# jianzhnie/ScaleRL

Measured on NVIDIA H100. Metric: learner_frames_per_sec, higher is better.
Workload: dtype bf16

## Files before the change

scalerl_b200/csrc/common.cuh:

```cuda
#pragma once
#include <cuda_runtime.h>
#include <cuda_bf16.h>
#include <stdint.h>
#include "wgmma.cuh"

#define SRL_DEVINL __device__ __forceinline__

#ifndef SRL_SPIN_LIMIT
#define SRL_SPIN_LIMIT (1u << 24)
#endif

namespace srl {

SRL_DEVINL uint32_t smem_u32(const void* p) { return static_cast<uint32_t>(__cvta_generic_to_shared(p)); }

SRL_DEVINL void mbar_init(uint64_t* bar, uint32_t count) {
  asm volatile("mbarrier.init.shared::cta.b64 [%0], %1;" ::"r"(smem_u32(bar)), "r"(count) : "memory");
}
SRL_DEVINL void mbar_fence_init() { asm volatile("fence.mbarrier_init.release.cluster;" ::: "memory"); }
SRL_DEVINL void mbar_arrive(uint64_t* bar) {
  asm volatile("{\n\t.reg .b64 st;\n\tmbarrier.arrive.shared::cta.b64 st, [%0];\n\t}" ::"r"(smem_u32(bar)) : "memory");
}
SRL_DEVINL void mbar_arrive_expect_tx(uint64_t* bar, uint32_t bytes) {
  asm volatile("{\n\t.reg .b64 st;\n\tmbarrier.arrive.expect_tx.shared::cta.b64 st, [%0], %1;\n\t}" ::"r"(smem_u32(bar)), "r"(bytes)
               : "memory");
}
SRL_DEVINL bool mbar_try_wait(uint64_t* bar, uint32_t parity) {
  uint32_t ok;
  asm volatile(
      "{\n\t.reg .pred p;\n\t"
      "mbarrier.try_wait.parity.shared::cta.b64 p, [%1], %2;\n\t"
      "selp.u32 %0, 1, 0, p;\n\t}"
      : "=r"(ok)
      : "r"(smem_u32(bar)), "r"(parity)
      : "memory");
  return ok != 0;
}
SRL_DEVINL void mbar_wait(uint64_t* bar, uint32_t parity) {
  uint32_t spins = 0;
  while (!mbar_try_wait(bar, parity)) {
    if (++spins > SRL_SPIN_LIMIT) { __trap(); }
  }
}

#ifdef SRL_KSTAMP
static __device__ unsigned long long* g_kstamp = nullptr;
SRL_DEVINL unsigned long long kstamp_now() { unsigned long long t; asm volatile("mov.u64 %0, %%globaltimer;" : "=l"(t)); return t; }
SRL_DEVINL void kstamp_put(int kid, unsigned long long t0) {
  if (g_kstamp && blockIdx.x == 0 && blockIdx.y == 0 && threadIdx.x == 0) {
    const unsigned long long t1 = kstamp_now(), i = atomicAdd(g_kstamp, 1ull);
    if (i < 2000) { g_kstamp[1 + 3 * i] = (unsigned long long)kid; g_kstamp[2 + 3 * i] = t0; g_kstamp[3 + 3 * i] = t1; }
  }
}
#define SRL_KSTAMP_SETTER(fn) void fn(unsigned long long* q) { cudaMemcpyToSymbol(g_kstamp, &q, sizeof q); }
#else
#define SRL_KSTAMP_SETTER(fn) void fn(unsigned long long*) {}
#endif
SRL_DEVINL void pdl_wait(int kid = 0) {
#ifdef SRL_KSTAMP
  const unsigned long long t0 = kstamp_now();
#endif
  asm volatile("griddepcontrol.wait;" ::: "memory");
#ifdef SRL_KSTAMP
  if (kid) kstamp_put(kid, t0);
#else
  (void)kid;
#endif
}
SRL_DEVINL void pdl_launch() { asm volatile("griddepcontrol.launch_dependents;" ::: "memory"); }

SRL_DEVINL uint4 lds128(uint32_t saddr) {
  uint4 v;
  asm volatile("ld.shared.v4.b32 {%0, %1, %2, %3}, [%4];" : "=r"(v.x), "=r"(v.y), "=r"(v.z), "=r"(v.w) : "r"(saddr) : "memory");
  return v;
}
SRL_DEVINL void sts_volatile_f32(uint32_t saddr, float v) { asm volatile("st.volatile.shared.f32 [%0], %1;" ::"r"(saddr), "f"(v) : "memory"); }

SRL_DEVINL void fence_proxy_async_smem() { asm volatile("fence.proxy.async.shared::cta;" ::: "memory"); }

SRL_DEVINL uint32_t elect_one_sync() {
  uint32_t pred;
  __syncwarp();
  asm volatile("{\n\t.reg .pred P;\n\telect.sync _|P, 0xffffffff;\n\tselp.u32 %0, 1, 0, P;\n\t}" : "=r"(pred));
  return pred;
}
SRL_DEVINL void wg_fence() { asm volatile("wgmma.fence.sync.aligned;" ::: "memory"); }
SRL_DEVINL void wg_commit() { asm volatile("wgmma.commit_group.sync.aligned;" ::: "memory"); }
SRL_DEVINL void wg_wait_all() { asm volatile("wgmma.wait_group.sync.aligned 0;" ::: "memory"); }
SRL_DEVINL void wg_wait_prev() { asm volatile("wgmma.wait_group.sync.aligned 1;" ::: "memory"); }
template <int N> SRL_DEVINL void reg_release() { asm volatile("setmaxnreg.dec.sync.aligned.u32 %0;" ::"n"(N)); }
template <int N> SRL_DEVINL void reg_claim() { asm volatile("setmaxnreg.inc.sync.aligned.u32 %0;" ::"n"(N)); }
template <int N>
SRL_DEVINL void wg_fence_regs(float (&d)[N]) {
#pragma unroll
  for (int i = 0; i < N; ++i) asm volatile("" : "+f"(d[i])::"memory");
}
SRL_DEVINL void named_bar(int id, int threads) { asm volatile("bar.sync %0, %1;" ::"r"(id), "r"(threads) : "memory"); }

template <int N, int TA, int TB>
SRL_DEVINL void wg_mma128(float (&d)[2][N / 2], uint64_t ad, uint32_t a_hi, uint64_t bd, uint32_t accumulate) {
  Wgmma<N, TA, TB>::mma(d[0], ad, bd, accumulate);
  Wgmma<N, TA, TB>::mma(d[1], ad + a_hi, bd, accumulate);
}

constexpr int fit_stages(int want, int fixed, int per) {
  int s = want;
  while (s > 1 && fixed + s * per > 232448) --s;
  return s;
}
constexpr int WG_IMG_STRIDE = 20;
constexpr int WG_IMG_BYTES = 2 * 128 * WG_IMG_STRIDE * 4;
template <int N, bool ONE_BUF = false>
SRL_DEVINL void wg_acc_rows16(const float (&d0)[N / 2], const float (&d1)[N / 2], int c, float* img, int wt, int bar, float (&v)[16]) {
  float* buf = ONE_BUF ? img : img + (c & 1) * 128 * WG_IMG_STRIDE;
  if (ONE_BUF) named_bar(bar, 128);
  const int w = wt >> 5, l = wt & 31;
#pragma unroll
  for (int h = 0; h < 2; ++h)
#pragma unroll
    for (int jj = 0; jj < 2; ++jj)
#pragma unroll
      for (int rr = 0; rr < 2; ++rr) {
        const int row = 64 * h + 16 * w + (l >> 2) + 8 * rr, i = 4 * (2 * c + jj) + 2 * rr;
        const float (&d)[N / 2] = h ? d1 : d0;
        *reinterpret_cast<float2*>(buf + row * WG_IMG_STRIDE + 8 * jj + 2 * (l & 3)) = make_float2(d[i], d[i + 1]);
      }
  named_bar(bar, 128);
  const float4* q = reinterpret_cast<const float4*>(buf + wt * WG_IMG_STRIDE);
#pragma unroll
  for (int j = 0; j < 4; ++j) { const float4 x = q[j]; v[4 * j] = x.x; v[4 * j + 1] = x.y; v[4 * j + 2] = x.z; v[4 * j + 3] = x.w; }
}
template <int N, bool ONE_BUF = false>
SRL_DEVINL void wg_acc_row16(const float (&d)[2][N / 2], int c, float* img, int wt, int bar, float (&v)[16]) {
  wg_acc_rows16<N, ONE_BUF>(d[0], d[1], c, img, wt, bar, v);
}

SRL_DEVINL uint64_t make_smem_desc(uint32_t saddr, uint32_t lbo_bytes, uint32_t sbo_bytes) {
  uint64_t d = 0;
  d |= (uint64_t)((saddr & 0x3FFFF) >> 4);
  d |= (uint64_t)((lbo_bytes >> 4) & 0x3FFF) << 16;
  d |= (uint64_t)((sbo_bytes >> 4) & 0x3FFF) << 32;
  d |= (uint64_t)1 << 62;
  return d;
}
SRL_DEVINL uint64_t make_smem_desc_sw64(uint32_t saddr, uint32_t lbo_bytes, uint32_t sbo_bytes) {
  return (make_smem_desc(saddr, lbo_bytes, sbo_bytes) & ~((uint64_t)3 << 62)) | ((uint64_t)2 << 62);
}

SRL_DEVINL uint32_t swz128(uint32_t row, uint32_t chunk) { return row * 128u + ((chunk ^ (row & 7u)) << 4); }
SRL_DEVINL uint32_t swz64(uint32_t row, uint32_t chunk) { return row * 64u + ((chunk ^ ((row >> 1) & 3u)) << 4); }

SRL_DEVINL uint32_t pack_bf16x2(float lo, float hi) {
  __nv_bfloat162 v = __floats2bfloat162_rn(lo, hi);
  return *reinterpret_cast<uint32_t*>(&v);
}
SRL_DEVINL float bf16_lo(uint32_t v) { return __uint_as_float(v << 16); }
SRL_DEVINL float bf16_hi(uint32_t v) { return __uint_as_float(v & 0xFFFF0000u); }

SRL_DEVINL void red_add_v4(float* addr, float a, float b, float c, float d) {
  asm volatile("red.global.add.v4.f32 [%0], {%1, %2, %3, %4};" ::"l"(addr), "f"(a), "f"(b), "f"(c), "f"(d) : "memory");
}
SRL_DEVINL void red_add_16(float* dst, const float (&v)[16], float scale = 1.0f) {
#pragma unroll
  for (int j = 0; j < 16; j += 4) red_add_v4(dst + j, v[j] * scale, v[j + 1] * scale, v[j + 2] * scale, v[j + 3] * scale);
}

SRL_DEVINL int ld_action(const int64_t* p, int A) {
  const long long a = __ldg(reinterpret_cast<const long long*>(p));
  return a < 0 ? 0 : (a >= A ? A - 1 : (int)a);
}

SRL_DEVINL float warp_sum(float v) {
#pragma unroll
  for (int o = 16; o > 0; o >>= 1) v += __shfl_xor_sync(0xffffffffu, v, o);
  return v;
}

SRL_DEVINL bool take_ticket(float* scratch) {
  __threadfence();
  return atomicAdd(reinterpret_cast<unsigned*>(scratch), 1u) == gridDim.x - 1;
}

}
```

scalerl_b200/csrc/encoder.cu:

```cuda
#include "encoder_problems.cuh"
#include "tma_problems.cuh"
#include "res_problems.cuh"
#include "enc_fused.cuh"
#include "kernels.h"
#include <stdio.h>
#include <stdlib.h>

namespace srl {

constexpr int PACK_BLOCKS_FK = 256, PACK_BLOCKS_FD = 256, PACK_BLOCKS_CONV = 288;
SRL_DEVINL void pack_store(bf16* __restrict__ out, bf16* __restrict__ out_lo, int64_t i, float v) {
  const bf16 hi = __float2bfloat16_rn(v);
  out[i] = hi;
  if (out_lo) out_lo[i] = __float2bfloat16_rn(v - __bfloat162float(hi));
}
SRL_DEVINL void pack_store2(bf16* __restrict__ out, bf16* __restrict__ out_lo, int64_t i, float v0, float v1) {
  const bf16 h0 = __float2bfloat16_rn(v0), h1 = __float2bfloat16_rn(v1);
  *reinterpret_cast<uint32_t*>(out + i) = pack_bf16x2(v0, v1);
  if (out_lo) *reinterpret_cast<uint32_t*>(out_lo + i) = pack_bf16x2(v0 - __bfloat162float(h0), v1 - __bfloat162float(h1));
}
__global__ void __launch_bounds__(256) pack_weights_kernel(ParamPtrs p, bf16* __restrict__ out, bf16* __restrict__ out_lo, int skip_w1k) {
  pdl_wait(2);
  __shared__ __align__(16) float tile[64 * 99];
  const int t = threadIdx.x, b = blockIdx.x;
// ... 44 lines not shown
      } else if (i < WPack::W3K) {
        const int e = (int)(i - WPack::W2K), co = e >> 9, k = e & 511, tap = k >> 5, c = k & 31;
        v = p.w2[((co * 32 + c) << 4) + tap];
      } else if (i < WPack::WFK) {
        const int e = (int)(i - WPack::W3K), co = e / 576, k = e - co * 576, tap = k >> 6, c = k & 63;
        v = p.w3[(co * 64 + c) * 9 + tap];
      } else if (i < WPack::W2D) {
        const int e = (int)(i - WPack::W3D), c = e / 576, k = e - c * 576, tap = k >> 6, co = k & 63;
        v = p.w3[(co * 64 + c) * 9 + tap];
      } else {
        const int e = (int)(i - WPack::W2D), cls = e >> 13, r = e & 8191, c = r >> 8, k = r & 255, tt = k >> 6, co = k & 63;
        const int kh = (cls >> 1) + 2 * (tt >> 1), kw = (cls & 1) + 2 * (tt & 1);
        v = p.w2[((co * 32 + c) << 4) + kh * 4 + kw];
      }
      pack_store(out, out_lo, i, v);
    }
  }
}

__global__ void __launch_bounds__(352) obs_s2d_kernel(const uint8_t* __restrict__ obs, bf16* __restrict__ xs, int frame_blocks,
                                                      const float* __restrict__ w1, bf16* __restrict__ w1k, bf16* __restrict__ w1k_lo) {
  pdl_wait(1);
  pdl_launch();
  if ((int)blockIdx.x >= frame_blocks) {
    const int e = ((int)blockIdx.x - frame_blocks) * 352 + (int)threadIdx.x;
    if (e < 32 * 256 && w1k) {
      const int co = e >> 8, k = e & 255, tap = k >> 6, q = k & 63;
      const int c = q >> 4, dy = (q >> 2) & 3, dx = q & 3, kh = 4 * (tap >> 1) + dy, kw = 4 * (tap & 1) + dx;
      pack_store(w1k, w1k_lo, e, __ldg(w1 + co * 256 + c * 64 + kh * 8 + kw));
    }
    return;
  }
  __shared__ uint32_t tile[21][16][21];
  const int n = blockIdx.x;
  const int t = threadIdx.x;
  if (t < 336) {
    const int g = t / 21, X = t - g * 21;
    const uint8_t* src = obs + (size_t)n * 28224 + (g >> 2) * 7056 + (g & 3) * 84;
#pragma unroll
    for (int y = 0; y < 21; ++y) tile[y][g][X] = __ldg(reinterpret_cast<const uint32_t*>(src + y * 336) + X);
  }
  __syncthreads();
  if (t < 336) {
    const int X = t >> 4, g = t & 15;
#pragma unroll
    for (int y = 0; y < 21; ++y) {
      const uint32_t w = tile[y][g][X];
      const float f0 = __uint_as_float(__byte_perm(w, 0x4B000000u, 0x7540)) - 8388608.f;
      const float f1 = __uint_as_float(__byte_perm(w, 0x4B000000u, 0x7541)) - 8388608.f;
      const float f2 = __uint_as_float(__byte_perm(w, 0x4B000000u, 0x7542)) - 8388608.f;
      const float f3 = __uint_as_float(__byte_perm(w, 0x4B000000u, 0x7543)) - 8388608.f;
      *reinterpret_cast<uint2*>(xs + (((size_t)n * 21 + y) * 21 + X) * 64 + g * 4) = make_uint2(pack_bf16x2(f0, f1), pack_bf16x2(f2, f3));
    }
  }
}

__global__ void __launch_bounds__(256) a3_transpose_kernel(const bf16* __restrict__ a3, bf16* __restrict__ a3t) {
  pdl_wait(53);
  __shared__ __align__(16) uint16_t tile[49 * 66];
  const int n = blockIdx.x, t = threadIdx.x;
  const uint4* src = reinterpret_cast<const uint4*>(a3 + (size_t)n * 3136);
  for (int q = t; q < 392; q += 256) {
    const uint4 v = __ldg(src + q);
    uint32_t* d = reinterpret_cast<uint32_t*>(tile + (q >> 3) * 66 + (q & 7) * 8);
    d[0] = v.x; d[1] = v.y; d[2] = v.z; d[3] = v.w;
  }
  __syncthreads();
  uint32_t* dst = reinterpret_cast<uint32_t*>(a3t + (size_t)n * 3136);
  for (int pp = t; pp < 1568; pp += 256) {
    const int o = 2 * pp, c0 = o / 49, h0 = o - c0 * 49, o1 = o + 1, c1 = o1 / 49, h1 = o1 - c1 * 49;
    dst[pp] = (uint32_t)tile[h0 * 66 + c0] | ((uint32_t)tile[h1 * 66 + c1] << 16);
  }
}
SRL_KSTAMP_SETTER(kstamp_set_encoder)

cudaError_t launch_a3_transpose(const bf16* a3, bf16* a3t, int frames, cudaStream_t st) {
  if (frames <= 0) return cudaSuccess;
  a3_transpose_kernel<<<frames, 256, 0, st>>>(a3, a3t);
  return cudaGetLastError();
}

cudaError_t launch_pack_weights(const ParamPtrs& p, bf16* wpack, cudaStream_t st, bf16* wpack_lo, bool skip_w1k) {
  pack_weights_kernel<<<PACK_BLOCKS_FK + PACK_BLOCKS_FD + PACK_BLOCKS_CONV, 256, 0, st>>>(p, wpack, wpack_lo, skip_w1k ? 1 : 0);
  return cudaGetLastError();
}

#define SRL_TRY(x) do { cudaError_t e_ = (x); if (e_ != cudaSuccess) return e_; } while (0)

static inline int cdiv(int a, int b) { return (a + b - 1) / b; }

typedef CUresult (*EncodeTiledFn)(CUtensorMap*, CUtensorMapDataType, cuuint32_t, void*, const cuuint64_t*, const cuuint64_t*,
                                  const cuuint32_t*, const cuuint32_t*, CUtensorMapInterleave, CUtensorMapSwizzle,
                                  CUtensorMapL2promotion, CUtensorMapFloatOOBfill);

static EncodeTiledFn encode_fn() {
  static EncodeTiledFn fn = nullptr;
  if (!fn) {
    void* f = nullptr;
    cudaDriverEntryPointQueryResult q;
    if (cudaGetDriverEntryPoint("cuTensorMapEncodeTiled", &f, cudaEnableDefault, &q) == cudaSuccess && q == cudaDriverEntryPointSuccess)
      fn = reinterpret_cast<EncodeTiledFn>(f);
  }
  return fn;
}

bool make_map(CUtensorMap* m, const void* base, int rank, const uint64_t* dims, const uint64_t* strides_elems, const uint32_t* box,
              bool swizzle64) {
  EncodeTiledFn fn = encode_fn();
  if (!fn) return false;
  cuuint64_t gd[5], gs[4];
  cuuint32_t bx[5], es[5];
  for (int i = 0; i < rank; ++i) { gd[i] = dims[i]; bx[i] = box[i]; es[i] = 1; }
  for (int i = 0; i + 1 < rank; ++i) gs[i] = strides_elems[i] * 2;
  return fn(m, CU_TENSOR_MAP_DATA_TYPE_BFLOAT16, (cuuint32_t)rank, const_cast<void*>(base), gd, gs, bx, es, CU_TENSOR_MAP_INTERLEAVE_NONE,
            swizzle64 ? CU_TENSOR_MAP_SWIZZLE_64B : CU_TENSOR_MAP_SWIZZLE_128B, CU_TENSOR_MAP_L2_PROMOTION_L2_128B,
            CU_TENSOR_MAP_FLOAT_OOB_FILL_NONE) == CUDA_SUCCESS;
}

struct MapBuilder {
  const char* failed = nullptr;
  bool lo = false, failed_lo = false;
  void operator()(CUtensorMap* m, const void* base, uint64_t inner, uint64_t rows, uint32_t box_inner, uint32_t box_rows, const char* name,
                  bool swizzle64 = false) {
    const uint64_t d[2] = {inner, rows}, s[1] = {inner};
    const uint32_t bx[2] = {box_inner, box_rows};
    if (!failed && !make_map(m, base, 2, d, s, bx, swizzle64)) { failed = name; failed_lo = lo; }
  }
};

static void build_operand_maps(MapBuilder& mk, const OperandTensors& b, uint64_t nf, uint64_t nb, OperandMaps* M) {
  mk(&M->a1p0_w, b.a1, 64, nf * 100, 64, RConv2Fwd::WROWS, "a1p0_w");
  mk(&M->a1p1_w, b.a1 + (size_t)nf * 100 * 64, 64, nf * 100, 64, RConv2Fwd::WROWS, "a1p1_w");
  mk(&M->a2_w, b.a2, 64, nf * 81, 64, RConv3Fwd::WROWS, "a2_w");
  mk(&M->da3g_w, b.da3, 64, nb * 81, 64, RConv3Dgrad::WROWS, "da3g_w");
  mk(&M->da3g_b, b.da3, 64, nb * 81, 64, 128, "da3g_b");
  mk(&M->da2g_w, b.da2, 64, nb * 100, 64, RConv2Dgrad::WROWS, "da2g_w");
  mk(&M->da2g_b, b.da2, 64, nb * 100, 64, 128, "da2g_b");
  mk(&M->da1g_b, b.da1, 32, nb * 441, 32, 128, "da1g_b", true);
  mk(&M->a3m128, b.a3, 3136, nf, 64, 128, "a3m128");
  mk(&M->a3m64, b.a3, 3136, nf, 64, 64, "a3m64");
  mk(&M->dhm128, b.dh, 512, nb, 64, 128, "dhm128");
  mk(&M->dhm64, b.dh, 512, nb, 64, 64, "dhm64");
  const bf16* w = b.wpack;
  mk(&M->w1k, w + WPack::W1K, 256, 32, 64, 32, "w1k");
  mk(&M->w2k, w + WPack::W2K, 512, 64, 64, 64, "w2k");
  mk(&M->w3k, w + WPack::W3K, 576, 64, 64, 64, "w3k");
  mk(&M->wfk, w + WPack::WFK, 3136, 512, 64, 64, "wfk");
  mk(&M->wfd, w + WPack::WFD, 512, 3136, 64, 64, "wfd");
  mk(&M->w3d, w + WPack::W3D, 576, 64, 64, 64, "w3d");
  mk(&M->w2d, w + WPack::W2D, 256, 128, 64, 128, "w2d");
}

cudaError_t build_tma_maps(const EncoderBuffers& b, int NF, int NB, TmaMaps* M, const char** why) {
  static_assert(RConv1Wgrad::WROWS == RConv1Fwd::WROWS && RConv2Wgrad::WROWS == RConv2Fwd::WROWS && RConv3Wgrad::WROWS == RConv3Fwd::WROWS,
                "forward and wgrad share the window maps");
  const uint64_t nf = NF, nb = NB;
  MapBuilder mk;
  mk(&M->xs_w, b.xs, 64, nf * 441, 64, RConv1Fwd::WROWS, "xs_w");
  mk(&M->a3tm64, b.a3t, 3136, nf, 64, 64, "a3tm64");
  build_operand_maps(mk, b.hi, nf, nb, &M->hi);
  mk.lo = true;
  if (b.lo.wpack) build_operand_maps(mk, b.lo, nf, nb, &M->lo);
  M->valid = !mk.failed;
  if (mk.failed && why) {
    static thread_local char name[32];
    snprintf(name, sizeof(name), "%s%s", mk.failed, mk.failed_lo ? "_lo" : "");
    *why = name;
  }
  return mk.failed ? cudaErrorInvalidValue : cudaSuccess;
}

static cudaError_t launch_s2d(const uint8_t* obs, int frames, bf16* xs, cudaStream_t st, const float* w1, bf16* w1k, bf16* w1k_lo) {
  constexpr int WB = (32 * 256 + 351) / 352;
  SRL_TRY(launch_chain(obs_s2d_kernel, dim3(frames + WB), dim3(352), 0, st, obs, xs, frames, w1, w1k, w1k_lo));
  return cudaGetLastError();
}

static int sm_count() {
  static const int n = [] { int d = 0, v = 0; cudaGetDevice(&d); cudaDeviceGetAttribute(&v, cudaDevAttrMultiProcessorCount, d); return v > 0 ? v : 132; }();
  return n;
}
static int persistent_ctas() {
  static int v = 0;
  if (!v) {
    const char* e = getenv("SRL_PERSISTENT_CTAS");
    v = e ? atoi(e) : sm_count();
    if (v < 16 || v > sm_count()) v = sm_count();
  }
  return v;
}
#define kPersistentCtas persistent_ctas()
static int bwd_ctas() {
  static const int v = [] { const char* e = getenv("SRL_BWD_CTAS"); int x = e ? atoi(e) : 0; return x < 16 || x > sm_count() ? 0 : x; }();
  return v ? v : persistent_ctas() - persistent_ctas() / 9;
}
static int side_wgrad_ctas() {
  static const int v = [] { const char* e = getenv("SRL_WGRAD_CTAS"); int x = e ? atoi(e) : 64; return x < 8 || x > sm_count() ? 64 : x; }();
  return v;
}

struct WgradReduce3 {
  static constexpr int KID = 0, CO = 64, BIAS = 64, PART = WSP_W3, NR = 18, ROW_GROUPS = 32;
  static constexpr bool FRAMES_U8 = false;
  SRL_DEVINL static int row(int rg, int i) { return (i % 9) * 64 + 2 * rg + i / 9; }
};
struct WgradReduce2 {
  static constexpr int KID = 0, CO = 64, BIAS = 64, PART = WSP_W2, NR = 16, ROW_GROUPS = 32;
  static constexpr bool FRAMES_U8 = false;
  SRL_DEVINL static int row(int rg, int i) { return (i >> 2) * 128 + (i & 3) * 32 + rg; }
};
struct WgradReduce1 {
  static constexpr int KID = 51, CO = 32, BIAS = 32, PART = WSP_W1, NR = 16, ROW_GROUPS = 16;
  static constexpr bool FRAMES_U8 = true;
  SRL_DEVINL static int row(int rg, int i) {
    const int c = rg >> 2, kh2 = (rg >> 1) & 1, dy = 2 * (rg & 1) + (i >> 3), kw = i & 7;
    return kh2 * 128 + (kw >> 2) * 64 + c * 16 + dy * 4 + (kw & 3);
  }
};
template <class L>
__global__ void __launch_bounds__(L::NR * 8) conv_wgrad_reduce_kernel(const float* __restrict__ part, int n, float* __restrict__ g,
                                                                       float* __restrict__ db) {
  constexpr int CG = L::CO / 8, TILES = L::ROW_GROUPS * CG;
  static_assert(L::BIAS <= 8 * L::NR, "the bias block fits the tile's threads and shared memory");
  extern __shared__ __align__(16) float stage[];
  pdl_wait(L::KID);
  pdl_launch();
  const int t = threadIdx.x, rg = blockIdx.x / CG, co0 = (blockIdx.x % CG) * 8;
  const bool bias = blockIdx.x == TILES;
  const int per = bias ? L::BIAS / 4 : 2 * L::NR;
  for (int k = t; k < n * per; k += L::NR * 8) {
    const int c = k / per, q = k - c * per;
    const float* src = part + (size_t)c * L::PART + (bias ? L::PART - L::BIAS + 4 * q : L::row(rg, q >> 1) * L::CO + co0 + 4 * (q & 1));
    asm volatile("cp.async.cg.shared.global [%0], [%1], 16;" ::"r"(smem_u32(stage + 4 * k)), "l"(src) : "memory");
  }
  asm volatile("cp.async.wait_all;" ::: "memory");
  __syncthreads();
  const int w = bias ? L::BIAS : 8 * L::NR;
  if (t >= w) return;
  float s = 0.f;
  for (int c = 0; c < n; ++c) s += stage[c * w + t];
  if (bias) db[t] += s;
  else g[(size_t)(co0 + (t & 7)) * (L::ROW_GROUPS * L::NR) + L::NR * rg + (t >> 3)] = L::FRAMES_U8 ? s * (1.0f / 255.0f) : s;
}

template <class L>
static cudaError_t launch_wgrad_reduce(const float* part, int n, float* g, float* db, cudaStream_t st) {
  static PerDeviceOnce once;
  SRL_TRY(ensure_max_dynamic_smem(once, conv_wgrad_reduce_kernel<L>, WG_PART_CTAS * L::NR * 32));
  static const int greatest = [] { int lo = 0, hi = 0; return cudaDeviceGetStreamPriorityRange(&lo, &hi) == cudaSuccess ? hi : 0; }();
  cudaLaunchConfig_t cfg = {};
  cfg.gridDim = dim3(L::ROW_GROUPS * (L::CO / 8) + 1); cfg.blockDim = dim3(L::NR * 8); cfg.dynamicSmemBytes = (size_t)n * L::NR * 32; cfg.stream = st;
  cudaLaunchAttribute attr[1];
  attr[0].id = cudaLaunchAttributePriority;
  attr[0].val.priority = greatest;
  cfg.attrs = attr; cfg.numAttrs = 1;
  return cudaLaunchKernelEx(&cfg, conv_wgrad_reduce_kernel<L>, part, n, g, db);
}

cudaError_t encoder_forward(const uint8_t* obs, int frames, const ParamPtrs& p, const EncoderBuffers& buf, const TmaMaps& maps, int mode,
                            const StepStreams& S, bool fused_front) {
  if (frames <= 0) return cudaSuccess;
  if ((mode != 0 && mode != 1) || !maps.valid) return cudaErrorInvalidValue;
  const int sp = mode;
  if (sp && !buf.lo.wpack) return cudaErrorInvalidValue;
  const cudaStream_t st = S.main;
  if (fused_front && !sp && (reinterpret_cast<uintptr_t>(obs) & 15) == 0) {
    EncFusedParams q{obs, p.w1, p.b1, p.w2, p.b2, buf.xs, buf.hi.a1, buf.hi.a2, frames, buf.NF};
    S.b(PS_ENC_FUSED); SRL_TRY(enc_fused_fwd_launch(q, kPersistentCtas, st)); S.e(PS_ENC_FUSED);
    SRL_TRY(S.join(LANE_PACK));
  } else {
  S.b(PS_S2D); SRL_TRY(launch_s2d(obs, frames, buf.xs, st, p.w1, buf.hi.wpack + WPack::W1K, sp ? buf.lo.wpack + WPack::W1K : nullptr)); S.e(PS_S2D);
  { RConv1Fwd::Params q{maps.xs_w, maps.hi.w1k, maps.lo.w1k, p.b1, buf.hi.a1, buf.lo.a1, frames, buf.NF};
    S.b(PS_CONV1_FWD); SRL_TRY(res_fwd_launch<RConv1Fwd>(q, cdiv(frames * 441, 128), kPersistentCtas, st, sp)); S.e(PS_CONV1_FWD); }
  SRL_TRY(S.join(LANE_PACK));
  { RConv2Fwd::Params q{maps.hi.a1p0_w, maps.hi.a1p1_w, maps.hi.w2k, maps.lo.a1p0_w, maps.lo.a1p1_w, maps.lo.w2k, p.b2, buf.hi.a2, buf.lo.a2, frames};
    S.b(PS_CONV2_FWD); SRL_TRY(res_fwd_launch<RConv2Fwd>(q, cdiv(frames * 100, 128), kPersistentCtas, st, sp)); S.e(PS_CONV2_FWD); }
  }
  { RConv3Fwd::Params q{maps.hi.a2_w, maps.hi.w3k, maps.lo.a2_w, maps.lo.w3k, p.b3, buf.hi.a3, buf.lo.a3, frames};
    S.b(PS_CONV3_FWD); SRL_TRY(res_fwd_launch<RConv3Fwd>(q, cdiv(frames * 81, 128), kPersistentCtas, st, sp)); S.e(PS_CONV3_FWD); }
  { TFcFwd::Params q{maps.hi.a3m128, maps.hi.wfk, maps.lo.a3m128, maps.lo.wfk, buf.hpart, frames};
    static_assert(TFcFwd::SPLITS == FC_SPLITS, "split count");
    S.b(PS_FC_FWD);
    if (sp) SRL_TRY((igemm_tma_launch<TFcFwd, 1>(q, dim3(cdiv(frames, 128), 8 * FC_SPLITS), st)));
    else SRL_TRY((igemm_tma_launch<TFcFwd, 0>(q, dim3(cdiv(frames, 128), 8 * FC_SPLITS), st)));
    S.e(PS_FC_FWD); }
  return cudaSuccess;
}

cudaError_t encoder_backward(int frames, const EncoderBuffers& buf, const ParamPtrs& g, const TmaMaps& maps, int mode,
                             const StepStreams& S, BwdParts parts, bool a3t_done) {
  if (frames <= 0) return cudaSuccess;
  if ((mode != 0 && mode != 1) || !maps.valid) return cudaErrorInvalidValue;
  const int sp = mode;
  if (sp && !buf.lo.wpack) return cudaErrorInvalidValue;
  const bool do_fc = parts & BWD_FC, do_conv = parts & BWD_CONV;
  const cudaStream_t st = S.main, s1 = S.lane(LANE_FC_WGRAD), s2 = S.lane(LANE_CONV3_WGRAD), s3 = S.lane(LANE_CONV2_WGRAD);
  if (do_fc) {
    SRL_TRY(S.fork(LANE_FC_WGRAD));
    { const bool native = !sp && buf.a3t != nullptr;
      S.b(PS_FC_WGRAD);
      if (native) {
        if (!a3t_done) SRL_TRY(launch_a3_transpose(buf.hi.a3, buf.a3t, frames, s1));
        TFcWgradN::Params q{maps.hi.dhm64, maps.a3tm64, g.wf, g.bf, frames};
        SRL_TRY((igemm_tma_launch<TFcWgradN, 0>(q, dim3(1, 4 * (TFcWgradN::NCT + 1)), s1)));
      } else {
        TFcWgrad::Params q{maps.hi.dhm64, maps.hi.a3m64, maps.lo.dhm64, maps.lo.a3m64, g.wf, g.bf, frames};
        if (sp) SRL_TRY((igemm_tma_launch<TFcWgrad, 1>(q, dim3(1, 4 * 50), s1))); else SRL_TRY((igemm_tma_launch<TFcWgrad, 0>(q, dim3(1, 4 * 50), s1)));
      }
      S.e(PS_FC_WGRAD); }
    { TFcDgrad::Params q{maps.hi.dhm128, maps.hi.wfd, maps.lo.dhm128, maps.lo.wfd, buf.hi.a3, buf.hi.da3, buf.lo.da3, frames};
      S.b(PS_FC_DGRAD);
      if (sp) SRL_TRY((igemm_tma_launch<TFcDgrad, 1>(q, dim3(cdiv(frames, 128), 49), st))); else SRL_TRY((igemm_tma_launch<TFcDgrad, 0>(q, dim3(cdiv(frames, 128), 49), st)));
      S.e(PS_FC_DGRAD); }
    if (!do_conv) SRL_TRY(S.join(LANE_FC_WGRAD));
  }
  if (!do_conv) return cudaSuccess;
  SRL_TRY(S.fork(LANE_CONV3_WGRAD));
  float* part3 = buf.wgrad_part;
  float* part2 = part3 + (size_t)WG_PART_CTAS * WSP_W3;
  float* part1 = part2 + (size_t)WG_PART_CTAS * WSP_W2;
  int n3 = 0, n2 = 0, n1 = 0;
  { RConv3Wgrad::Params q{maps.hi.a2_w, maps.hi.da3g_b, maps.lo.a2_w, maps.lo.da3g_b, part3, frames * 81, 0};
    S.b(PS_CONV3_WGRAD); SRL_TRY(res_wgrad_launch<RConv3Wgrad>(q, side_wgrad_ctas(), s2, &n3, sp)); S.e(PS_CONV3_WGRAD); }
  if (!S.collapsed) SRL_TRY(launch_wgrad_reduce<WgradReduce3>(part3, n3, g.w3, g.b3, s2));
  { RConv3Dgrad::Params q{maps.hi.da3g_w, maps.hi.w3d, maps.lo.da3g_w, maps.lo.w3d, buf.hi.a2, buf.hi.da2, buf.lo.da2, frames};
    S.b(PS_CONV3_DGRAD); SRL_TRY(res_fwd_launch<RConv3Dgrad>(q, cdiv(frames * 81, 128), bwd_ctas(), st, sp)); S.e(PS_CONV3_DGRAD); }
  SRL_TRY(S.fork(LANE_CONV2_WGRAD));
  { RConv2Wgrad::Params q{maps.hi.a1p0_w, maps.hi.a1p1_w, maps.hi.da2g_b, maps.lo.a1p0_w, maps.lo.a1p1_w, maps.lo.da2g_b, part2, frames * 100, 0};
    S.b(PS_CONV2_WGRAD); SRL_TRY(res_wgrad_launch<RConv2Wgrad>(q, side_wgrad_ctas(), s3, &n2, sp)); S.e(PS_CONV2_WGRAD); }
  if (!S.collapsed) SRL_TRY(launch_wgrad_reduce<WgradReduce2>(part2, n2, g.w2, g.b2, s3));
  { RConv2Dgrad::Params q{maps.hi.da2g_w, maps.hi.w2d, maps.lo.da2g_w, maps.lo.w2d, buf.hi.a1, buf.hi.da1, buf.lo.da1, frames, buf.NF};
    S.b(PS_CONV2_DGRAD); SRL_TRY(res_fwd_launch<RConv2Dgrad>(q, cdiv(frames * 100, 128), bwd_ctas(), st, sp)); S.e(PS_CONV2_DGRAD); }
  { RConv1Wgrad::Params q{maps.xs_w, maps.hi.da1g_b, maps.lo.da1g_b, part1, frames * 441, 0};
    S.b(PS_CONV1_WGRAD); SRL_TRY(res_wgrad_launch<RConv1Wgrad>(q, bwd_ctas(), st, &n1, sp)); S.e(PS_CONV1_WGRAD); }
  S.b(PS_WGRAD_FINALIZE);
  if (S.collapsed) {
    SRL_TRY(launch_wgrad_reduce<WgradReduce3>(part3, n3, g.w3, g.b3, st));
    SRL_TRY(launch_wgrad_reduce<WgradReduce2>(part2, n2, g.w2, g.b2, st));
  }
  SRL_TRY(launch_wgrad_reduce<WgradReduce1>(part1, n1, g.w1, g.b1, st));
  S.e(PS_WGRAD_FINALIZE);
  if (do_fc) SRL_TRY(S.join(LANE_FC_WGRAD));
  SRL_TRY(S.join(LANE_CONV3_WGRAD));
  SRL_TRY(S.join(LANE_CONV2_WGRAD));
  return cudaSuccess;
}

}
```

scalerl_b200/csrc/igemm_tma.cuh:

```cuda
#pragma once
#include <cuda.h>
#include "common.cuh"
#include "kernels.h"

namespace srl {

SRL_DEVINL void tma_prefetch_desc(const CUtensorMap* m) {
  asm volatile("prefetch.tensormap [%0];" ::"l"(reinterpret_cast<uint64_t>(m)) : "memory");
}
SRL_DEVINL void tma_load_2d(void* dst, const CUtensorMap* m, uint64_t* bar, int c0, int c1) {
  asm volatile("cp.async.bulk.tensor.2d.shared::cluster.global.mbarrier::complete_tx::bytes [%0], [%1, {%3, %4}], [%2];"
               ::"r"(smem_u32(dst)), "l"(reinterpret_cast<uint64_t>(m)), "r"(smem_u32(bar)), "r"(c0), "r"(c1) : "memory");
}
SRL_DEVINL void tma_load_3d(void* dst, const CUtensorMap* m, uint64_t* bar, int c0, int c1, int c2) {
  asm volatile("cp.async.bulk.tensor.3d.shared::cluster.global.mbarrier::complete_tx::bytes [%0], [%1, {%3, %4, %5}], [%2];"
               ::"r"(smem_u32(dst)), "l"(reinterpret_cast<uint64_t>(m)), "r"(smem_u32(bar)), "r"(c0), "r"(c1), "r"(c2) : "memory");
}
SRL_DEVINL void tma_load_4d(void* dst, const CUtensorMap* m, uint64_t* bar, int c0, int c1, int c2, int c3) {
  asm volatile("cp.async.bulk.tensor.4d.shared::cluster.global.mbarrier::complete_tx::bytes [%0], [%1, {%3, %4, %5, %6}], [%2];"
               ::"r"(smem_u32(dst)), "l"(reinterpret_cast<uint64_t>(m)), "r"(smem_u32(bar)), "r"(c0), "r"(c1), "r"(c2), "r"(c3)
               : "memory");
}
SRL_DEVINL void tma_load_5d(void* dst, const CUtensorMap* m, uint64_t* bar, int c0, int c1, int c2, int c3, int c4) {
  asm volatile("cp.async.bulk.tensor.5d.shared::cluster.global.mbarrier::complete_tx::bytes [%0], [%1, {%3, %4, %5, %6, %7}], [%2];"
               ::"r"(smem_u32(dst)), "l"(reinterpret_cast<uint64_t>(m)), "r"(smem_u32(bar)), "r"(c0), "r"(c1), "r"(c2), "r"(c3), "r"(c4)
               : "memory");
}

constexpr int IGT_THREADS = 288;

template <class P, int SPLIT = 0>
struct TmaCfg {
  static constexpr int KROWS = P::A_MN ? P::KROWS : 64;
  static constexpr int A_BYTES = P::A_MN ? 2 * KROWS * 128 : 128 * 128;
  static constexpr int B_BLOCKS = (P::BN + 63) / 64;
  static constexpr int B_BYTES = P::B_MN ? B_BLOCKS * KROWS * 128 : P::BN * 128;
  static constexpr int HALF_BYTES = A_BYTES + B_BYTES;
  static constexpr int STAGE_BYTES = HALF_BYTES * (1 + SPLIT);
  static constexpr int NB = P::BN / 2;
  static constexpr int STAGES = fit_stages(P::STAGES, 2 * WG_IMG_BYTES + 1024 + 256, STAGE_BYTES);
  static constexpr int SMEM_BYTES = STAGES * STAGE_BYTES + 2 * WG_IMG_BYTES + 1024 + 256;
  static_assert(SMEM_BYTES <= 232448, "shared memory budget (227 KB)");
  static_assert(NB == 32 || NB == 64 || NB == 128, "MMA N per warpgroup");
  static constexpr int MMAS = P::A_MN ? KROWS / 16 : 4;
  static_assert(A_BYTES % 1024 == 0 && B_BYTES % 1024 == 0, "operand tiles must keep 1024 B alignment (SWIZZLE_128B atoms)");
  static_assert(P::A_MN == P::B_MN, "mixed majors are not used");
  static_assert(KROWS % 16 == 0, "contraction rows per stage must be a multiple of MMA K = 16");
};

template <class P, int SPLIT>
SRL_DEVINL void igt_epilogue(const typename P::Params& p, int tm, int ty, int row, int c0, float (&v)[16]) {
  if constexpr (SPLIT) P::template epilogue16<1>(p, tm, ty, row, c0, v); else P::epilogue16(p, tm, ty, row, c0, v);
}
template <class P, int SPLIT>
SRL_DEVINL void igt_epilogue(const typename P::Params& p, int tm, int ty, int row, int c0, float (&v)[16], const uint4 (&pre)[2]) {
  if constexpr (SPLIT) P::template epilogue16<1>(p, tm, ty, row, c0, v, pre); else P::epilogue16(p, tm, ty, row, c0, v, pre);
}

template <class P, int SPLIT = 0>
__global__ void __launch_bounds__(IGT_THREADS) igemm_tma_kernel(const __grid_constant__ typename P::Params p) {
  using C = TmaCfg<P, SPLIT>;
  extern __shared__ uint8_t smem_raw[];
  uint8_t* smem = reinterpret_cast<uint8_t*>((reinterpret_cast<uintptr_t>(smem_raw) + 1023) & ~uintptr_t(1023));
  float* img = reinterpret_cast<float*>(smem + C::STAGES * C::STAGE_BYTES);
  uint64_t* bars = reinterpret_cast<uint64_t*>(smem + C::STAGES * C::STAGE_BYTES + 2 * WG_IMG_BYTES);
  uint64_t* full = bars;
  uint64_t* empty = bars + C::STAGES;

  const int tid = threadIdx.x;
  const int warp = tid >> 5;
  const int tm = blockIdx.x, ty = blockIdx.y;
  const int nkb = P::num_kblocks(p, tm, ty);

  if constexpr (P::ZERO_INIT) {
    if (P::zero_cta(ty)) {
      uint4* z = reinterpret_cast<uint4*>(smem);
      for (int i = tid; i < C::STAGES * C::STAGE_BYTES / 16; i += IGT_THREADS) z[i] = make_uint4(0, 0, 0, 0);
    }
    __syncthreads();
    for (int s = 0; s < C::STAGES; ++s) P::init_smem(p, tm, ty, smem + s * C::STAGE_BYTES, tid);
    fence_proxy_async_smem();
  }
  if (warp == 8 && (tid & 31) == 0) {
    for (int s = 0; s < C::STAGES; ++s) { mbar_init(&full[s], 1); mbar_init(&empty[s], 8); }
    mbar_fence_init();
    P::prefetch(p);
  }
  __syncthreads();
  pdl_wait(P::KID);
  if (tid == 256) pdl_launch();

  if (warp == 8) {
    const uint32_t leader = elect_one_sync();
    for (int kb = 0; kb < nkb; ++kb) {
      const int s = kb % C::STAGES;
      mbar_wait(&empty[s], ((kb / C::STAGES) & 1) ^ 1);
      if (leader) {
        uint8_t* sA = smem + s * C::STAGE_BYTES;
        if constexpr (SPLIT) P::issue_split(p, tm, ty, kb, sA, C::A_BYTES, C::HALF_BYTES, &full[s]);
        else P::issue(p, tm, ty, kb, sA, sA + C::A_BYTES, &full[s]);
      }
      __syncwarp();
    }
  } else {
    const int g = warp >> 2, wt = tid & 127;
    constexpr int NB = C::NB;
    uint4 pre[P::PREFETCH ? NB / 16 : 1][2];
    if constexpr (P::PREFETCH) {
#pragma unroll
      for (int c = 0; c < NB / 16; ++c) P::prefetch16(p, tm, ty, wt, g * NB + c * 16, pre[c]);
    }
    float acc[2][NB / 2];
#pragma unroll
    for (int h = 0; h < 2; ++h)
#pragma unroll
      for (int i = 0; i < NB / 2; ++i) acc[h][i] = 0.f;
    constexpr uint32_t ASTEP = P::A_MN ? 2048 / 16 : 32 / 16, BSTEP = P::B_MN ? 2048 / 16 : 32 / 16;
    constexpr uint32_t A_HI = (P::A_MN ? C::KROWS * 128 : 64 * 128) / 16;
    const uint32_t b_off = P::B_MN ? (g * NB / 64) * C::KROWS * 128 + (g * NB % 64) * 2 : g * NB * 128;
    for (int kb = 0; kb < nkb; ++kb) {
      const int s = kb % C::STAGES;
      mbar_wait(&full[s], (kb / C::STAGES) & 1);
      const uint32_t a0 = smem_u32(smem + s * C::STAGE_BYTES);
      const uint64_t ad0 = P::A_MN ? make_smem_desc(a0, C::KROWS * 128, 1024) : make_smem_desc(a0, 16, 1024);
      const uint64_t bd0 = P::B_MN ? make_smem_desc(a0 + C::A_BYTES + b_off, C::KROWS * 128, 1024) : make_smem_desc(a0 + C::A_BYTES + b_off, 16, 1024);
      wg_fence();
#pragma unroll
      for (int k = 0; k < C::MMAS; ++k) {
        const uint64_t ad = ad0 + (uint64_t)(k * ASTEP), bd = bd0 + (uint64_t)(k * BSTEP);
        wg_mma128<NB, P::A_MN ? 1 : 0, P::B_MN ? 1 : 0>(acc, ad, A_HI, bd, (kb | k) != 0);
        if constexpr (SPLIT) {
          wg_mma128<NB, P::A_MN ? 1 : 0, P::B_MN ? 1 : 0>(acc, ad, A_HI, bd + (uint64_t)(C::HALF_BYTES / 16), 1);
          wg_mma128<NB, P::A_MN ? 1 : 0, P::B_MN ? 1 : 0>(acc, ad + (uint64_t)(C::HALF_BYTES / 16), A_HI, bd, 1);
        }
      }
      wg_commit();
      if constexpr (C::STAGES > 1) {
        wg_wait_prev();
        __syncwarp();
        if (kb > 0 && (tid & 31) == 0) mbar_arrive(&empty[(kb - 1) % C::STAGES]);
      } else {
        wg_wait_all();
        __syncwarp();
        if ((tid & 31) == 0) mbar_arrive(&empty[s]);
      }
    }
    wg_wait_all();
    wg_fence_regs(acc[0]); wg_fence_regs(acc[1]);
    float* my_img = img + g * (WG_IMG_BYTES / 4);
#pragma unroll
    for (int c = 0; c < NB / 16; ++c) {
      float v[16];
      wg_acc_row16<NB>(acc, c, my_img, wt, 2 + g, v);
      if constexpr (P::PREFETCH) igt_epilogue<P, SPLIT>(p, tm, ty, wt, g * NB + c * 16, v, pre[c]);
      else igt_epilogue<P, SPLIT>(p, tm, ty, wt, g * NB + c * 16, v);
    }
  }
}

template <class P, int SPLIT = 0>
cudaError_t igemm_tma_launch(const typename P::Params& p, dim3 grid, cudaStream_t stream) {
  using C = TmaCfg<P, SPLIT>;
  if (grid.x == 0 || grid.y == 0) return cudaSuccess;
  static PerDeviceOnce once;
  { cudaError_t e = ensure_max_dynamic_smem(once, igemm_tma_kernel<P, SPLIT>, C::SMEM_BYTES); if (e != cudaSuccess) return e; }
  return launch_chain(igemm_tma_kernel<P, SPLIT>, grid, dim3(IGT_THREADS), C::SMEM_BYTES, stream, p);
}

}
```

scalerl_b200/csrc/tma_problems.cuh:

```cuda
#pragma once
#include "igemm_tma.cuh"
#include "encoder_problems.cuh"

namespace srl {

#define SRL_TMAP alignas(64) CUtensorMap

struct TFcFwd {
  static constexpr int KID = 31;
  static constexpr bool PREFETCH = false;
  static constexpr int BN = 64, STAGES = 4, SPLITS = 4;
  static constexpr bool A_MN = false, B_MN = false, ZERO_INIT = false;
  static constexpr int KROWS = 64;
  struct Params { SRL_TMAP a3m; SRL_TMAP w; SRL_TMAP a3m_lo; SRL_TMAP w_lo; float* out; int M; };
  SRL_DEVINL static void prefetch(const Params& p) { tma_prefetch_desc(&p.a3m); tma_prefetch_desc(&p.w); }
  SRL_DEVINL static int kb_begin(int split) { return (49 * split) / SPLITS; }
  SRL_DEVINL static void issue_split(const Params& p, int tm, int ty, int kb, uint8_t* st, int a_bytes, int half, uint64_t* bar) {
    const int k = (kb_begin(ty % SPLITS) + kb) * 64;
    mbar_arrive_expect_tx(bar, 2 * (128 * 128 + 64 * 128));
    tma_load_2d(st, &p.a3m, bar, k, tm * 128);
    tma_load_2d(st + a_bytes, &p.w, bar, k, (ty / SPLITS) * 64);
    tma_load_2d(st + half, &p.a3m_lo, bar, k, tm * 128);
    tma_load_2d(st + half + a_bytes, &p.w_lo, bar, k, (ty / SPLITS) * 64);
  }
  template <int SPLIT>
  SRL_DEVINL static void epilogue16(const Params& p, int tm, int ty, int row, int c0, float (&v)[16]) { epilogue16(p, tm, ty, row, c0, v); }
  SRL_DEVINL static int num_kblocks(const Params&, int, int ty) { const int sp = ty % SPLITS; return kb_begin(sp + 1) - kb_begin(sp); }
  SRL_DEVINL static void issue(const Params& p, int tm, int ty, int kb, uint8_t* sA, uint8_t* sB, uint64_t* bar) {
    const int k = (kb_begin(ty % SPLITS) + kb) * 64;
    mbar_arrive_expect_tx(bar, 128 * 128 + 64 * 128);
    tma_load_2d(sA, &p.a3m, bar, k, tm * 128);
    tma_load_2d(sB, &p.w, bar, k, (ty / SPLITS) * 64);
  }
  SRL_DEVINL static void epilogue16(const Params& p, int tm, int ty, int row, int c0, float (&v)[16]) {
    const int m = tm * 128 + row;
    if (m >= p.M) return;
    float4* o = reinterpret_cast<float4*>(p.out + ((size_t)(ty % SPLITS) * p.M + m) * 512 + (ty / SPLITS) * 64 + c0);
#pragma unroll
    for (int j = 0; j < 4; ++j) o[j] = make_float4(v[4 * j], v[4 * j + 1], v[4 * j + 2], v[4 * j + 3]);
  }
};

struct TFcDgrad {
  static constexpr int KID = 32;
  static constexpr bool PREFETCH = true;
  static constexpr int BN = 64, STAGES = 4;
  static constexpr bool A_MN = false, B_MN = false, ZERO_INIT = false;
  static constexpr int KROWS = 64;
  struct Params { SRL_TMAP dhm; SRL_TMAP w; SRL_TMAP dhm_lo; SRL_TMAP w_lo; const bf16* a3; bf16* da3; bf16* da3_lo; int M; };
  SRL_DEVINL static void prefetch(const Params& p) { tma_prefetch_desc(&p.dhm); tma_prefetch_desc(&p.w); }
  SRL_DEVINL static int num_kblocks(const Params&, int, int) { return 8; }
  SRL_DEVINL static void issue_split(const Params& p, int tm, int ty, int kb, uint8_t* st, int a_bytes, int half, uint64_t* bar) {
    mbar_arrive_expect_tx(bar, 2 * (128 * 128 + 64 * 128));
    tma_load_2d(st, &p.dhm, bar, kb * 64, tm * 128);
    tma_load_2d(st + a_bytes, &p.w, bar, kb * 64, ty * 64);
    tma_load_2d(st + half, &p.dhm_lo, bar, kb * 64, tm * 128);
    tma_load_2d(st + half + a_bytes, &p.w_lo, bar, kb * 64, ty * 64);
  }
  SRL_DEVINL static void issue(const Params& p, int tm, int ty, int kb, uint8_t* sA, uint8_t* sB, uint64_t* bar) {
    mbar_arrive_expect_tx(bar, 128 * 128 + 64 * 128);
    tma_load_2d(sA, &p.dhm, bar, kb * 64, tm * 128);
    tma_load_2d(sB, &p.w, bar, kb * 64, ty * 64);
  }
  SRL_DEVINL static void prefetch16(const Params& p, int tm, int ty, int row, int c0, uint4 (&mk)[2]) {
    const int m = tm * 128 + row;
    if (m < p.M) ld_mask16(p.a3 + (size_t)m * 3136 + ty * 64 + c0, mk);
  }
  SRL_DEVINL static void epilogue16(const Params& p, int tm, int ty, int row, int c0, float (&v)[16], const uint4 (&mk)[2]) {
    epilogue16<0>(p, tm, ty, row, c0, v, mk);
  }
  template <int SPLIT>
  SRL_DEVINL static void epilogue16(const Params& p, int tm, int ty, int row, int c0, float (&v)[16], const uint4 (&mk)[2]) {
    const int m = tm * 128 + row;
    if (m >= p.M) return;
    relu_mask16_pre(mk, v);
    const size_t o = ((size_t)m * 81 + (ty / 7) * 9 + ty % 7) * 64 + c0;
    store_bf16x16(p.da3 + o, v);
    if constexpr (SPLIT) {
      float r[16];
#pragma unroll
      for (int j = 0; j < 16; ++j) r[j] = v[j] - __bfloat162float(__float2bfloat16_rn(v[j]));
      store_bf16x16(p.da3_lo + o, r);
    }
  }
};

SRL_DEVINL void fill_ones(uint8_t* dst, int bytes, int tid) {
  uint4* q = reinterpret_cast<uint4*>(dst);
  for (int i = tid; i < bytes / 16; i += IGT_THREADS) q[i] = make_uint4(0x3F803F80u, 0x3F803F80u, 0x3F803F80u, 0x3F803F80u);
}

struct TFcWgrad {
  static constexpr int KID = 33;
  static constexpr bool PREFETCH = false;
  static constexpr int BN = 64, STAGES = 4, KROWS = 64;
  static constexpr bool A_MN = true, B_MN = true, ZERO_INIT = true;
  struct Params { SRL_TMAP dhm; SRL_TMAP a3m; SRL_TMAP dhm_lo; SRL_TMAP a3m_lo; float* dw; float* db; int M; };
  SRL_DEVINL static void prefetch(const Params& p) { tma_prefetch_desc(&p.dhm); tma_prefetch_desc(&p.a3m); }
  SRL_DEVINL static void issue_split(const Params& p, int, int ty, int kb, uint8_t* st, int a_bytes, int half, uint64_t* bar) {
    const int hw = ty >> 2, j0 = (ty & 3) * 128;
    mbar_arrive_expect_tx(bar, (hw < 49 ? 6 : 4) * 64 * 128);
    tma_load_2d(st, &p.dhm, bar, j0, kb * 64);
    tma_load_2d(st + KROWS * 128, &p.dhm, bar, j0 + 64, kb * 64);
    tma_load_2d(st + half, &p.dhm_lo, bar, j0, kb * 64);
    tma_load_2d(st + half + KROWS * 128, &p.dhm_lo, bar, j0 + 64, kb * 64);
    if (hw < 49) {
      tma_load_2d(st + a_bytes, &p.a3m, bar, hw * 64, kb * 64);
      tma_load_2d(st + half + a_bytes, &p.a3m_lo, bar, hw * 64, kb * 64);
    }
  }
  template <int SPLIT>
  SRL_DEVINL static void epilogue16(const Params& p, int tm, int ty, int row, int c0, float (&v)[16]) { epilogue16(p, tm, ty, row, c0, v); }
  SRL_DEVINL static bool zero_cta(int) { return true; }
  SRL_DEVINL static int num_kblocks(const Params& p, int, int) { return (p.M + 63) >> 6; }
  SRL_DEVINL static void init_smem(const Params&, int, int ty, uint8_t* stage, int tid) {
    if ((ty >> 2) == 49) fill_ones(stage + 2 * KROWS * 128, KROWS * 128, tid);
  }
  SRL_DEVINL static void issue(const Params& p, int, int ty, int kb, uint8_t* sA, uint8_t* sB, uint64_t* bar) {
    const int hw = ty >> 2, j0 = (ty & 3) * 128;
    mbar_arrive_expect_tx(bar, (hw < 49 ? 3 : 2) * 64 * 128);
    tma_load_2d(sA, &p.dhm, bar, j0, kb * 64);
    tma_load_2d(sA + KROWS * 128, &p.dhm, bar, j0 + 64, kb * 64);
    if (hw < 49) tma_load_2d(sB, &p.a3m, bar, hw * 64, kb * 64);
  }
  SRL_DEVINL static void epilogue16(const Params& p, int, int ty, int row, int c0, float (&v)[16]) {
    const int j = (ty & 3) * 128 + row, hw = ty >> 2;
    if (hw < 49) {
#pragma unroll
      for (int jj = 0; jj < 16; ++jj) p.dw[(size_t)j * 3136 + (c0 + jj) * 49 + hw] = v[jj];
    } else if (c0 == 0) {
      p.db[j] = v[0];
    }
  }
};

struct TFcWgradN {
  static constexpr int KID = 36;
  static constexpr bool PREFETCH = false;
  static constexpr int BN = 256, STAGES = 4, KROWS = 64, NCT = 13;
  static constexpr bool A_MN = true, B_MN = true, ZERO_INIT = true;
  struct Params { SRL_TMAP dhm; SRL_TMAP a3tm; float* dw; float* db; int M; };
  SRL_DEVINL static void prefetch(const Params& p) { tma_prefetch_desc(&p.dhm); tma_prefetch_desc(&p.a3tm); }
  SRL_DEVINL static bool zero_cta(int ty) { return (ty >> 2) == NCT; }
  SRL_DEVINL static int num_kblocks(const Params& p, int, int) { return (p.M + 63) >> 6; }
  SRL_DEVINL static void init_smem(const Params&, int, int ty, uint8_t* stage, int tid) {
    if ((ty >> 2) == NCT) fill_ones(stage + 2 * KROWS * 128, KROWS * 128, tid);
  }
  SRL_DEVINL static void issue(const Params& p, int, int ty, int kb, uint8_t* sA, uint8_t* sB, uint64_t* bar) {
    const int ct = ty >> 2, j0 = (ty & 3) * 128;
    const int nb = ct < NCT ? (ct == NCT - 1 ? 1 : 4) : 0;
    mbar_arrive_expect_tx(bar, (2 + nb) * 64 * 128);
    tma_load_2d(sA, &p.dhm, bar, j0, kb * 64);
    tma_load_2d(sA + KROWS * 128, &p.dhm, bar, j0 + 64, kb * 64);
    for (int q = 0; q < nb; ++q) tma_load_2d(sB + q * KROWS * 128, &p.a3tm, bar, ct * 256 + q * 64, kb * 64);
  }
  SRL_DEVINL static void epilogue16(const Params& p, int, int ty, int row, int c0, float (&v)[16]) {
    const int j = (ty & 3) * 128 + row, ct = ty >> 2, col = ct * 256 + c0;
    if (ct < NCT) {
      if (col < 3136) {
        float4* d = reinterpret_cast<float4*>(p.dw + (size_t)j * 3136 + col);
#pragma unroll
        for (int q = 0; q < 4; ++q) d[q] = make_float4(v[4 * q], v[4 * q + 1], v[4 * q + 2], v[4 * q + 3]);
      }
    } else if (c0 == 0) {
      p.db[j] = v[0];
    }
  }
};

}
```

Measured before the change: 2.518 million.

## Retile FC weight-grad to BN=128 with coalesced smem tile-store epilogue

The native FC weight-gradient GEMM moves from 256-wide to 128-wide column tiles (25 column tiles instead of 13+1). The bias column is folded into the last tile's ones-padding instead of a separate zero CTA. The epilogue now dumps the whole accumulator into the drained stage ring, then writes coalesced float4 rows to global memory instead of per-thread 16-float rows through the image buffer. This frees the image smem and aims at better store coalescing and SM fill. Separately, the conv2 dgrad launch uses the persistent CTA count instead of bwd_ctas(), which may change the concurrency balance with side streams.

```diff
diff --git a/scalerl_b200/csrc/common.cuh b/scalerl_b200/csrc/common.cuh
--- a/scalerl_b200/csrc/common.cuh
+++ b/scalerl_b200/csrc/common.cuh
@@ -134,6 +134,19 @@
 SRL_DEVINL void wg_acc_row16(const float (&d)[2][N / 2], int c, float* img, int wt, int bar, float (&v)[16]) {
   wg_acc_rows16<N, ONE_BUF>(d[0], d[1], c, img, wt, bar, v);
 }
+template <int N>
+SRL_DEVINL void wg_acc_to_tile(const float (&d)[2][N / 2], float* tile, int stride, int wt) {
+  const int w = wt >> 5, l = wt & 31;
+#pragma unroll
+  for (int h = 0; h < 2; ++h)
+#pragma unroll
+    for (int j = 0; j < N / 8; ++j)
+#pragma unroll
+      for (int rr = 0; rr < 2; ++rr) {
+        const int row = 64 * h + 16 * w + (l >> 2) + 8 * rr;
+        *reinterpret_cast<float2*>(tile + row * stride + 8 * j + 2 * (l & 3)) = make_float2(d[h][4 * j + 2 * rr], d[h][4 * j + 2 * rr + 1]);
+      }
+}
 
 SRL_DEVINL uint64_t make_smem_desc(uint32_t saddr, uint32_t lbo_bytes, uint32_t sbo_bytes) {
   uint64_t d = 0;
diff --git a/scalerl_b200/csrc/encoder.cu b/scalerl_b200/csrc/encoder.cu
--- a/scalerl_b200/csrc/encoder.cu
+++ b/scalerl_b200/csrc/encoder.cu
@@ -370,7 +370,7 @@
       if (native) {
         if (!a3t_done) SRL_TRY(launch_a3_transpose(buf.hi.a3, buf.a3t, frames, s1));
         TFcWgradN::Params q{maps.hi.dhm64, maps.a3tm64, g.wf, g.bf, frames};
-        SRL_TRY((igemm_tma_launch<TFcWgradN, 0>(q, dim3(1, 4 * (TFcWgradN::NCT + 1)), s1)));
+        SRL_TRY((igemm_tma_launch<TFcWgradN, 0>(q, dim3(1, 4 * TFcWgradN::NCT), s1)));
       } else {
         TFcWgrad::Params q{maps.hi.dhm64, maps.hi.a3m64, maps.lo.dhm64, maps.lo.a3m64, g.wf, g.bf, frames};
         if (sp) SRL_TRY((igemm_tma_launch<TFcWgrad, 1>(q, dim3(1, 4 * 50), s1))); else SRL_TRY((igemm_tma_launch<TFcWgrad, 0>(q, dim3(1, 4 * 50), s1)));
@@ -398,7 +398,7 @@
     S.b(PS_CONV2_WGRAD); SRL_TRY(res_wgrad_launch<RConv2Wgrad>(q, side_wgrad_ctas(), s3, &n2, sp)); S.e(PS_CONV2_WGRAD); }
   if (!S.collapsed) SRL_TRY(launch_wgrad_reduce<WgradReduce2>(part2, n2, g.w2, g.b2, s3));
   { RConv2Dgrad::Params q{maps.hi.da2g_w, maps.hi.w2d, maps.lo.da2g_w, maps.lo.w2d, buf.hi.a1, buf.hi.da1, buf.lo.da1, frames, buf.NF};
-    S.b(PS_CONV2_DGRAD); SRL_TRY(res_fwd_launch<RConv2Dgrad>(q, cdiv(frames * 100, 128), bwd_ctas(), st, sp)); S.e(PS_CONV2_DGRAD); }
+    S.b(PS_CONV2_DGRAD); SRL_TRY(res_fwd_launch<RConv2Dgrad>(q, cdiv(frames * 100, 128), kPersistentCtas, st, sp)); S.e(PS_CONV2_DGRAD); }
   { RConv1Wgrad::Params q{maps.xs_w, maps.hi.da1g_b, maps.lo.da1g_b, part1, frames * 441, 0};
     S.b(PS_CONV1_WGRAD); SRL_TRY(res_wgrad_launch<RConv1Wgrad>(q, bwd_ctas(), st, &n1, sp)); S.e(PS_CONV1_WGRAD); }
   S.b(PS_WGRAD_FINALIZE);
diff --git a/scalerl_b200/csrc/igemm_tma.cuh b/scalerl_b200/csrc/igemm_tma.cuh
--- a/scalerl_b200/csrc/igemm_tma.cuh
+++ b/scalerl_b200/csrc/igemm_tma.cuh
@@ -1,5 +1,6 @@
 #pragma once
 #include <cuda.h>
+#include <type_traits>
 #include "common.cuh"
 #include "kernels.h"
 
@@ -29,6 +30,9 @@
 
 constexpr int IGT_THREADS = 288;
 
+template <class P, class = void> struct TileStore : std::false_type {};
+template <class P> struct TileStore<P, std::void_t<decltype(P::TILE_STORE)>> : std::bool_constant<P::TILE_STORE> {};
+
 template <class P, int SPLIT = 0>
 struct TmaCfg {
   static constexpr int KROWS = P::A_MN ? P::KROWS : 64;
@@ -38,9 +42,13 @@
   static constexpr int HALF_BYTES = A_BYTES + B_BYTES;
   static constexpr int STAGE_BYTES = HALF_BYTES * (1 + SPLIT);
   static constexpr int NB = P::BN / 2;
-  static constexpr int STAGES = fit_stages(P::STAGES, 2 * WG_IMG_BYTES + 1024 + 256, STAGE_BYTES);
-  static constexpr int SMEM_BYTES = STAGES * STAGE_BYTES + 2 * WG_IMG_BYTES + 1024 + 256;
+  static constexpr bool TILE_STORE = TileStore<P>::value;
+  static constexpr int TILE_STRIDE = NB + 8;
+  static constexpr int IMG_BYTES = TILE_STORE ? 0 : 2 * WG_IMG_BYTES;
+  static constexpr int STAGES = fit_stages(P::STAGES, IMG_BYTES + 1024 + 256, STAGE_BYTES);
+  static constexpr int SMEM_BYTES = STAGES * STAGE_BYTES + IMG_BYTES + 1024 + 256;
   static_assert(SMEM_BYTES <= 232448, "shared memory budget (227 KB)");
+  static_assert(!TILE_STORE || 2 * 128 * TILE_STRIDE * 4 <= STAGES * STAGE_BYTES, "both accumulator tiles fit the stage ring");
   static_assert(NB == 32 || NB == 64 || NB == 128, "MMA N per warpgroup");
   static constexpr int MMAS = P::A_MN ? KROWS / 16 : 4;
   static_assert(A_BYTES % 1024 == 0 && B_BYTES % 1024 == 0, "operand tiles must keep 1024 B alignment (SWIZZLE_128B atoms)");
@@ -63,7 +71,7 @@
   extern __shared__ uint8_t smem_raw[];
   uint8_t* smem = reinterpret_cast<uint8_t*>((reinterpret_cast<uintptr_t>(smem_raw) + 1023) & ~uintptr_t(1023));
   float* img = reinterpret_cast<float*>(smem + C::STAGES * C::STAGE_BYTES);
-  uint64_t* bars = reinterpret_cast<uint64_t*>(smem + C::STAGES * C::STAGE_BYTES + 2 * WG_IMG_BYTES);
+  uint64_t* bars = reinterpret_cast<uint64_t*>(smem + C::STAGES * C::STAGE_BYTES + C::IMG_BYTES);
   uint64_t* full = bars;
   uint64_t* empty = bars + C::STAGES;
 
@@ -147,13 +155,21 @@
     }
     wg_wait_all();
     wg_fence_regs(acc[0]); wg_fence_regs(acc[1]);
-    float* my_img = img + g * (WG_IMG_BYTES / 4);
+    if constexpr (C::TILE_STORE) {
+      named_bar(1, 256);
+      float* tile = reinterpret_cast<float*>(smem) + g * 128 * C::TILE_STRIDE;
+      wg_acc_to_tile<NB>(acc, tile, C::TILE_STRIDE, wt);
+      named_bar(2 + g, 128);
+      P::store_tile(p, tm, ty, g, tile, C::TILE_STRIDE, wt);
+    } else {
+      float* my_img = img + g * (WG_IMG_BYTES / 4);
 #pragma unroll
-    for (int c = 0; c < NB / 16; ++c) {
-      float v[16];
-      wg_acc_row16<NB>(acc, c, my_img, wt, 2 + g, v);
-      if constexpr (P::PREFETCH) igt_epilogue<P, SPLIT>(p, tm, ty, wt, g * NB + c * 16, v, pre[c]);
-      else igt_epilogue<P, SPLIT>(p, tm, ty, wt, g * NB + c * 16, v);
+      for (int c = 0; c < NB / 16; ++c) {
+        float v[16];
+        wg_acc_row16<NB>(acc, c, my_img, wt, 2 + g, v);
+        if constexpr (P::PREFETCH) igt_epilogue<P, SPLIT>(p, tm, ty, wt, g * NB + c * 16, v, pre[c]);
+        else igt_epilogue<P, SPLIT>(p, tm, ty, wt, g * NB + c * 16, v);
+      }
     }
   }
 }
diff --git a/scalerl_b200/csrc/tma_problems.cuh b/scalerl_b200/csrc/tma_problems.cuh
--- a/scalerl_b200/csrc/tma_problems.cuh
+++ b/scalerl_b200/csrc/tma_problems.cuh
@@ -136,34 +136,36 @@
 
 struct TFcWgradN {
   static constexpr int KID = 36;
-  static constexpr bool PREFETCH = false;
-  static constexpr int BN = 256, STAGES = 4, KROWS = 64, NCT = 13;
+  static constexpr bool PREFETCH = false, TILE_STORE = true;
+  static constexpr int BN = 128, STAGES = 4, KROWS = 64, NCT = 25;
   static constexpr bool A_MN = true, B_MN = true, ZERO_INIT = true;
   struct Params { SRL_TMAP dhm; SRL_TMAP a3tm; float* dw; float* db; int M; };
   SRL_DEVINL static void prefetch(const Params& p) { tma_prefetch_desc(&p.dhm); tma_prefetch_desc(&p.a3tm); }
-  SRL_DEVINL static bool zero_cta(int ty) { return (ty >> 2) == NCT; }
+  SRL_DEVINL static bool zero_cta(int) { return false; }
   SRL_DEVINL static int num_kblocks(const Params& p, int, int) { return (p.M + 63) >> 6; }
   SRL_DEVINL static void init_smem(const Params&, int, int ty, uint8_t* stage, int tid) {
-    if ((ty >> 2) == NCT) fill_ones(stage + 2 * KROWS * 128, KROWS * 128, tid);
+    if ((ty >> 2) == NCT - 1) fill_ones(stage + 3 * KROWS * 128, KROWS * 128, tid);
   }
   SRL_DEVINL static void issue(const Params& p, int, int ty, int kb, uint8_t* sA, uint8_t* sB, uint64_t* bar) {
     const int ct = ty >> 2, j0 = (ty & 3) * 128;
-    const int nb = ct < NCT ? (ct == NCT - 1 ? 1 : 4) : 0;
+    const int nb = ct < NCT - 1 ? 2 : 1;
     mbar_arrive_expect_tx(bar, (2 + nb) * 64 * 128);
     tma_load_2d(sA, &p.dhm, bar, j0, kb * 64);
     tma_load_2d(sA + KROWS * 128, &p.dhm, bar, j0 + 64, kb * 64);
-    for (int q = 0; q < nb; ++q) tma_load_2d(sB + q * KROWS * 128, &p.a3tm, bar, ct * 256 + q * 64, kb * 64);
+    for (int q = 0; q < nb; ++q) tma_load_2d(sB + q * KROWS * 128, &p.a3tm, bar, ct * 128 + q * 64, kb * 64);
   }
-  SRL_DEVINL static void epilogue16(const Params& p, int, int ty, int row, int c0, float (&v)[16]) {
-    const int j = (ty & 3) * 128 + row, ct = ty >> 2, col = ct * 256 + c0;
-    if (ct < NCT) {
-      if (col < 3136) {
-        float4* d = reinterpret_cast<float4*>(p.dw + (size_t)j * 3136 + col);
-#pragma unroll
-        for (int q = 0; q < 4; ++q) d[q] = make_float4(v[4 * q], v[4 * q + 1], v[4 * q + 2], v[4 * q + 3]);
+  SRL_DEVINL static void store_tile(const Params& p, int, int ty, int g, const float* tile, int stride, int wt) {
+    const int j0 = (ty & 3) * 128, col = (ty >> 2) * 128 + g * 64;
+    if (col < 3136) {
+      const int w = wt >> 5, l = wt & 31;
+#pragma unroll 4
+      for (int i = 0; i < 16; ++i) {
+        const int r = 8 * i + 2 * w + (l >> 4);
+        const float4 v = *reinterpret_cast<const float4*>(tile + r * stride + 4 * (l & 15));
+        *reinterpret_cast<float4*>(p.dw + (size_t)(j0 + r) * 3136 + col + 4 * (l & 15)) = v;
       }
-    } else if (c0 == 0) {
-      p.db[j] = v[0];
+    } else {
+      p.db[j0 + wt] = tile[wt * stride];
     }
   }
 };
```

Result: faster. 2.562 million, median of 6 (+1.8%).
